# xingyizhou/CenterTrack

Hardware: AMD Instinct MI355X
Metric: frames/sec (DLA-34 + DCNv2 CenterTrack hot path: H2D of the frame + forward + decode + D2H + track association) (higher is better)
Workload: dtype f32; 1 GPU; mot17_512: mot heads, DLA-34, 512x512, 1 stream(s)/GPU, K=100, flip_test=False, seeded random-init weights; one step = 64 consecutive frames of every stream, each frame uploaded from pinned host memory inside the step (frame t+1 on a copy stream while frame t runs); global_batch=1, parallelism=streams sharded dp1, all-gather of packed detections, hip_graph=True

## Files before the change

centertrack_amd/_lib.py:

```python
import ctypes
import os

_PKG = os.path.dirname(os.path.abspath(__file__))
LIB_PATH = os.environ.get('CENTERTRACK_LIB') or os.path.join(_PKG, 'libcentertrack_hip.so')

c_float_p = ctypes.c_void_p
NUM_HEADS = 11
(HEAD_REG, HEAD_WH, HEAD_TRACKING, HEAD_LTRB, HEAD_LTRB_AMODAL, HEAD_DEP, HEAD_ROT, HEAD_DIM,
 HEAD_AMODEL_OFFSET, HEAD_NUSCENES_ATT, HEAD_VELOCITY) = range(NUM_HEADS)
HEAD_INDEX = {'reg': HEAD_REG, 'wh': HEAD_WH, 'tracking': HEAD_TRACKING, 'ltrb': HEAD_LTRB,
              'ltrb_amodal': HEAD_LTRB_AMODAL, 'dep': HEAD_DEP, 'rot': HEAD_ROT, 'dim': HEAD_DIM,
              'amodel_offset': HEAD_AMODEL_OFFSET, 'nuscenes_att': HEAD_NUSCENES_ATT,
              'velocity': HEAD_VELOCITY}
HEAD_CH = {'reg': 2, 'wh': 2, 'tracking': 2, 'ltrb': 4, 'ltrb_amodal': 4, 'dep': 1, 'rot': 8, 'dim': 3,
           'amodel_offset': 2, 'nuscenes_att': 8, 'velocity': 3}

CT_RELU = 1
CT_OUT_NCHW = 2
CT_DCN_MAIN, CT_DCN_FINISH, CT_DCN_OFFSETS = 1, 2, 4
CT_OK, CT_ERR_ARG, CT_ERR_LAUNCH, CT_ERR_WORKSPACE = 0, 1, 2, 3


class ConvDesc(ctypes.Structure):
    _fields_ = [('x', ctypes.c_void_p), ('N', ctypes.c_int), ('H', ctypes.c_int), ('W', ctypes.c_int),
                ('Cin', ctypes.c_int), ('ldx', ctypes.c_int),
                ('w_packed', ctypes.c_void_p), ('Cout', ctypes.c_int), ('ks', ctypes.c_int),
                ('stride', ctypes.c_int),
                ('scale', ctypes.c_void_p), ('shift', ctypes.c_void_p),
                ('res', ctypes.c_void_p), ('ldr', ctypes.c_int),
                ('y', ctypes.c_void_p), ('ldy', ctypes.c_int),
                ('flags', ctypes.c_int),
                ('sig_lo', ctypes.c_int), ('sig_hi', ctypes.c_int),
                ('dep_lo', ctypes.c_int), ('dep_hi', ctypes.c_int), ('depth_scale', ctypes.c_float),
                ('workspace', ctypes.c_void_p), ('workspace_bytes', ctypes.c_size_t),
                ('split_k', ctypes.c_int), ('algo', ctypes.c_int), ('w_winograd', ctypes.c_void_p),
                ('pool_y', ctypes.c_void_p), ('pool_ld', ctypes.c_int),
                ('proj_w_packed', ctypes.c_void_p), ('proj_scale', ctypes.c_void_p), ('proj_shift', ctypes.c_void_p),
                ('proj_y', ctypes.c_void_p), ('proj_ldy', ctypes.c_int)]


class DcnDesc(ctypes.Structure):
    _fields_ = [('x', ctypes.c_void_p), ('N', ctypes.c_int), ('H', ctypes.c_int), ('W', ctypes.c_int),
                ('Cin', ctypes.c_int), ('ldx', ctypes.c_int),
                ('om', ctypes.c_void_p), ('ldom', ctypes.c_int),
                ('w_packed', ctypes.c_void_p), ('Cout', ctypes.c_int),
                ('scale', ctypes.c_void_p), ('shift', ctypes.c_void_p),
                ('y', ctypes.c_void_p), ('ldy', ctypes.c_int),
                ('flags', ctypes.c_int),
                ('workspace', ctypes.c_void_p), ('workspace_bytes', ctypes.c_size_t),
                ('split_k', ctypes.c_int), ('algo', ctypes.c_int), ('fuse_offset', ctypes.c_int),
                ('w_off_packed', ctypes.c_void_p), ('b_off', ctypes.c_void_p),
                ('up_w', ctypes.c_void_p), ('up_f', ctypes.c_int), ('up_skip', ctypes.c_void_p), ('up_lds', ctypes.c_int),
                ('up_y', ctypes.c_void_p), ('up_ldy', ctypes.c_int),
                ('om_partial', ctypes.c_void_p), ('om_partial_bytes', ctypes.c_size_t),
                ('w_off_winograd', ctypes.c_void_p)]


CT_DCN_BWD_INPUT, CT_DCN_BWD_OFFSET_MASK, CT_DCN_BWD_WEIGHT = 1, 2, 4


class DcnBwdDesc(ctypes.Structure):
# ... 182 lines not shown
                ('inp_w', ctypes.c_int), ('inp_h', ctypes.c_int),
                ('host_rows', ctypes.c_void_p), ('rows_keep', ctypes.c_void_p),
                ('blob_params', ctypes.c_void_p), ('blob_counts', ctypes.c_void_p), ('blob_cap', ctypes.c_int),
                ('nslots', ctypes.c_int),
                ('graphs', ctypes.c_void_p * 3), ('frames', ctypes.c_void_p * 3),
                ('frame_bytes', ctypes.c_size_t),
                ('stream', ctypes.c_void_p),
                ('results', ctypes.c_void_p), ('results_cap', ctypes.c_int), ('done_flag', ctypes.c_void_p),
                ('pre', PrestageDesc)]


class FrameStepArgs(ctypes.Structure):
    _fields_ = [('slot', ctypes.c_int), ('frame_kind', ctypes.c_int),
                ('frame', ctypes.c_void_p), ('next_frame', ctypes.c_void_p),
                ('trans_input', ctypes.c_void_p), ('trans_inv', ctypes.c_void_p)]


CT_FRAME_DEVICE, CT_FRAME_HOST, CT_FRAME_IN_PLACE, CT_FRAME_UPLOADED = range(4)


ABI_VERSION = 103

EXPORTS = ['ct_last_error', 'ct_version', 'ct_set_tuning', 'ct_packed_weight_elems', 'ct_pack_conv_weight',
           'ct_packed_winograd_elems', 'ct_pack_winograd_weight', 'ct_conv2d',
           'ct_conv2d_workspace_bytes', 'ct_heads_fused', 'ct_dcn_v2', 'ct_dcn_v2_workspace_bytes', 'ct_dcn_v2_offsets_bytes', 'ct_dcn_v2_group', 'ct_dcn_v2_group_workspace_bytes', 'ct_dcn_v2_group_plan',
           'ct_dcn_v2_backward', 'ct_dcn_v2_backward_workspace_bytes', 'ct_packed_dcn_weight_t_elems', 'ct_pack_dcn_weight_t',
           'ct_generic_loss_forward', 'ct_generic_loss_backward', 'ct_generic_loss_workspace_bytes',
           'ct_conv2d_backward_weight', 'ct_conv2d_backward_weight_workspace_bytes', 'ct_heads_tail_backward',
           'ct_heads_tail_backward_workspace_bytes', 'ct_bn_stats', 'ct_bn_relu_apply', 'ct_bn_relu_backward', 'ct_bn_workspace_bytes',
           'ct_upsample_add_backward', 'ct_upsample_add_backward_workspace_bytes', 'ct_dcn_mask_sigmoid_backward',
           'ct_conv2d_s2_backward', 'ct_conv2d_s2_backward_workspace_bytes', 'ct_packed_conv_weight_s2t_elems', 'ct_pack_conv_weight_s2t',
           'ct_bn_act_apply', 'ct_bn_act_backward', 'ct_bn_act_workspace_bytes', 'ct_maxpool2x2_backward', 'ct_stem_forward',
           'ct_maxpool2x2', 'ct_upsample_add', 'ct_nchw_to_nhwc', 'ct_nhwc_to_nchw',
           'ct_decode_row_floats', 'ct_decode_workspace_bytes', 'ct_decode', 'ct_decode_pose_workspace_bytes',
           'ct_decode_pose', 'ct_render_pre_hm',
           'ct_tracker_create', 'ct_tracker_destroy', 'ct_tracker_reset', 'ct_tracker_num_tracks',
           'ct_tracker_id_count', 'ct_tracker_get_tracks', 'ct_tracker_step', 'ct_tracker_prehm_params', 'ct_linear_assignment', 'ct_tracker_set_mode', 'ct_tracker_init_tracks',
           'ct_tracker_step_public', 'ct_tracker_step_dets', 'ct_transform_points',
           'ct_preprocess_image', 'ct_preprocess_lut', 'ct_preprocess_device', 'ct_graph_begin', 'ct_graph_end', 'ct_graph_launch', 'ct_graph_destroy',
           'ct_memcpy_async', 'ct_memset_async', 'ct_stream_synchronize', 'ct_flip_merge', 'ct_flip_images',
           'ct_frame_loop_create', 'ct_frame_loop_destroy', 'ct_frame_loop_submit', 'ct_frame_loop_wait', 'ct_frame_loop_finish',
           'ct_frame_loop_finish_submit', 'ct_frame_loop_upload', 'ct_frame_loop_pending_slot', 'ct_frame_loop_in_flight',
           'ct_frame_loop_forget_upload', 'ct_frame_loop_prestage', 'ct_stem_forward_parts', 'ct_signal_host']

_lib = None


# ... 4 lines not shown
def load():
    global _lib
    if _lib is not None:
        return _lib
    if not os.path.exists(LIB_PATH):
        raise CTError('%s not found: build it with `python -c "import __graft_entry__ as g; g.build()"` '
                      '(hipcc --offload-arch=gfx950); there is no CPU fallback' % LIB_PATH)
    import torch
    lib = ctypes.CDLL(LIB_PATH)
    i, p, sz = ctypes.c_int, ctypes.c_void_p, ctypes.c_size_t
    lib.ct_last_error.restype = ctypes.c_char_p
    lib.ct_version.restype = i
    if lib.ct_version() != ABI_VERSION:
        raise CTError('%s is ABI version %d, this binding was written against %d: rebuild it (python -m '
                      'centertrack_amd.build)' % (LIB_PATH, lib.ct_version(), ABI_VERSION))
    lib.ct_set_tuning.argtypes = [ctypes.c_char_p, i]
    lib.ct_packed_weight_elems.restype = sz
    lib.ct_packed_weight_elems.argtypes = [i, i, i]
    lib.ct_pack_conv_weight.argtypes = [p, p, i, i, i, p]
    lib.ct_packed_winograd_elems.restype = sz
    lib.ct_packed_winograd_elems.argtypes = [i, i]
    lib.ct_pack_winograd_weight.argtypes = [p, p, i, i, p]
    lib.ct_conv2d.argtypes = [ctypes.POINTER(ConvDesc), p]
    lib.ct_conv2d_workspace_bytes.restype = sz
    lib.ct_conv2d_workspace_bytes.argtypes = [ctypes.POINTER(ConvDesc)]
    lib.ct_heads_fused.argtypes = [ctypes.POINTER(HeadsDesc), p]
    lib.ct_dcn_v2.argtypes = [ctypes.POINTER(DcnDesc), p]
    lib.ct_dcn_v2_workspace_bytes.restype = sz
    lib.ct_dcn_v2_workspace_bytes.argtypes = [ctypes.POINTER(DcnDesc)]
    lib.ct_dcn_v2_offsets_bytes.restype = sz
    lib.ct_dcn_v2_offsets_bytes.argtypes = [ctypes.POINTER(DcnDesc)]
    lib.ct_dcn_v2_group.argtypes = [ctypes.POINTER(DcnDesc), i, i, p]
    lib.ct_dcn_v2_group_workspace_bytes.restype = sz
    lib.ct_dcn_v2_group_workspace_bytes.argtypes = [ctypes.POINTER(DcnDesc)]
    lib.ct_dcn_v2_group_plan.argtypes = [ctypes.POINTER(DcnDesc), ctypes.POINTER(ctypes.c_size_t), ctypes.POINTER(ctypes.c_int)]
    lib.ct_dcn_v2_backward.argtypes = [ctypes.POINTER(DcnBwdDesc), p]
    lib.ct_dcn_v2_backward_workspace_bytes.restype = sz
    lib.ct_dcn_v2_backward_workspace_bytes.argtypes = [ctypes.POINTER(DcnBwdDesc)]
    lib.ct_packed_dcn_weight_t_elems.restype = sz
    lib.ct_packed_dcn_weight_t_elems.argtypes = [i, i]
    lib.ct_pack_dcn_weight_t.argtypes = [p, p, i, i, p]
    lib.ct_generic_loss_forward.argtypes = [ctypes.POINTER(LossDesc), p]
    lib.ct_generic_loss_backward.argtypes = [ctypes.POINTER(LossDesc), p]
    lib.ct_generic_loss_workspace_bytes.restype = sz
    lib.ct_generic_loss_workspace_bytes.argtypes = [ctypes.POINTER(LossDesc)]
    lib.ct_conv2d_backward_weight.argtypes = [ctypes.POINTER(ConvBwdWeightDesc), p]
# ... 124 lines not shown
```

centertrack_amd/csrc/conv_mfma.hip:

```cpp
#include "ct_common.h"
#define CT_KS_STAMP(i) CT_STAMP(i)
#include "ksplit_core.h"

CT_DEFINE_STAMPS(conv)

namespace {

struct ConvArgs {
    const float *x;
    const float *wp;
    int N, H, W, Cin, ldx;
    int tilesX, tilesY, coutBlocks, xcdPer;
    int NT;
    int nchunks;
    int chunksPerSplit;
    float *ws;
    int wsCout;
    EpiArgs epi;
    float *pool_y;
    int pool_ld;
    const float *proj_wp;
    EpiArgs epi2;
};

// ... 321 lines not shown
                const size_t Mtot = (size_t)a.N * a.epi.Ho * a.epi.Wo;
                float *wsp = a.ws + (size_t)split * Mtot * a.wsCout;
                const int co = (nt0 + nt) * 16 + li;
                if (oy < a.epi.Ho && co < a.wsCout) {
#pragma unroll
                    for (int e = 0; e < 4; ++e) {
                        const int ox = ox0 + lg * 4 + e;
                        if (ox < a.epi.Wo) wsp[(((size_t)n * a.epi.Ho + oy) * a.epi.Wo + ox) * a.wsCout + co] = sum[e];
                    }
                }
            } else {
                ct_store_tile(a.epi, sum, n, oy, ox0, (nt0 + nt) * 16, lane, psc[j], psh[j]);
            }
        };
    if constexpr (POOL && KS == 3 && STRIDE == 2) {
        auto fin_proj = [&](int mt, int nt, f32x4 sum, int j) {
            ct_store_tile(a.epi2, sum, n, oy0 + mt, ox0, (nt0 + nt) * 16, lane, psc2[j], psh2[j]);
        };
        ksplit_conv_tile<KS, STRIDE, WM, WN, WK, 2>(xin, a.H, a.W, a.ldx, a.Cin, a.wp, a.NT, nt0, oy0, ox0, c_begin, c_end, lds,
                                                    fin_main, hook, a.proj_wp, fin_proj);
    } else {
        ksplit_conv_tile<KS, STRIDE, WM, WN, WK, 2>(xin, a.H, a.W, a.ldx, a.Cin, a.wp, a.NT, nt0, oy0, ox0, c_begin, c_end, lds,
                                                    fin_main, hook);
    }
    CT_STAMP(6);
    CT_STAMP_RT(7);
}

__global__ __launch_bounds__(256) void splitk_reduce_kernel(const float *ws, int splits, size_t Mtot, int wsCout,
                                                            int N, EpiArgs e)
{
    const size_t idx = (size_t)blockIdx.x * 256 + threadIdx.x;
    const int quads = wsCout >> 2;
    if (idx >= Mtot * quads) return;
    const size_t m = idx / quads;
    const int c4 = (int)(idx - m * quads) << 2;
    f32x4 s = *reinterpret_cast<const f32x4 *>(ws + m * wsCout + c4);
    for (int k = 1; k < splits; ++k) {
        const f32x4 t = *reinterpret_cast<const f32x4 *>(ws + ((size_t)k * Mtot + m) * wsCout + c4);
        s += t;
    }
    const size_t hw = (size_t)e.Ho * e.Wo;
    const int n = (int)(m / hw);
    const size_t p = m - (size_t)n * hw;
#pragma unroll
    for (int i = 0; i < 4; ++i) {
// ... 246 lines not shown
extern "C" int ct_pack_conv_weight(const float *w_oihw, float *packed, int Cout, int Cin, int ks, void *stream)
{
    if (!w_oihw || !packed) CT_FAIL_ARG("ct_pack_conv_weight: null pointer");
    if (Cin % 16 || Cin <= 0 || Cout <= 0 || ks <= 0) CT_FAIL_ARG("ct_pack_conv_weight: Cin=%d must be a multiple of 16", Cin);
    const size_t total = ct_packed_weight_elems(Cout, Cin, ks);
    hipLaunchKernelGGL(pack_weight_kernel, dim3((unsigned)((total + 255) / 256)), dim3(256), 0, (hipStream_t)stream,
                       w_oihw, packed, Cout, Cin, ks, ct_cdiv(Cout, 16));
    CT_CHECK_LAUNCH("ct_pack_conv_weight");
    return CT_OK;
}

extern "C" size_t ct_conv2d_workspace_bytes(const ct_conv_desc *d)
{
    if (d && d->algo >= 201 && d->algo <= 211) return 0;
    Plan p;
    ct_conv_desc t = *d;
    float dummy;
    if (!t.workspace) t.workspace = &dummy;
    if (!t.y) t.y = &dummy;
    if (make_plan(&t, &p) != CT_OK) return 0;
    return ws_bytes(&t, p);
}

int ct_conv2d_winograd(const ct_conv_desc *d, void *stream);

extern "C" int ct_conv2d(const ct_conv_desc *d, void *stream)
{
    if (d && d->algo >= 201 && d->algo <= 211) {
        if (!d->x || !d->y) CT_FAIL_ARG("ct_conv2d: null pointer");
        if (d->ldx % 4 || ((uintptr_t)d->x & 15)) CT_FAIL_ARG("ct_conv2d: input view must be 16-byte aligned (ld %% 4 == 0)");
        return ct_conv2d_winograd(d, stream);
    }
    Plan p;
    int rc = make_plan(d, &p);
    if (rc != CT_OK) return rc;
    const size_t need = ws_bytes(d, p);
    if (need > 0 && (!d->workspace || d->workspace_bytes < need)) {
        ct_set_error("ct_conv2d: split_k=%d needs %zu workspace bytes, got %zu", p.splits, need, d->workspace_bytes);
        return CT_ERR_WORKSPACE;
    }
    if ((d->flags & CT_OUT_NCHW) && d->res) CT_FAIL_ARG("ct_conv2d: residual with NCHW output unsupported");
    ConvArgs a;
    a.x = d->x; a.wp = d->w_packed;
    a.N = d->N; a.H = d->H; a.W = d->W; a.Cin = d->Cin; a.ldx = d->ldx;
    a.tilesX = p.tilesX; a.tilesY = p.tilesY; a.coutBlocks = p.coutBlocks; a.xcdPer = ct_xcd_per(p.coutBlocks);
    a.NT = p.NT; a.nchunks = p.nchunks; a.chunksPerSplit = p.chunksPerSplit;
// ... 54 lines not shown
```

centertrack_amd/model.py:

```python
import ctypes
import os
from collections import OrderedDict

import torch

from . import _lib, autotune, ops
from .ops import View
from .weights import CHANNELS, LEVELS, dla34_param_shapes

BN_EPS = 1e-5
SMALL_SLOT_WGS = 600
FUSE_OFFSET = os.environ.get('CENTERTRACK_FUSE_OFFSET', '1') != '0'
WINOGRAD = os.environ.get('CENTERTRACK_WINOGRAD', '1') != '0'
FUSE_HEADS = os.environ.get('CENTERTRACK_FUSE_HEADS', '1') != '0'
FOLD_POOL = os.environ.get('CENTERTRACK_FOLD_POOL', '1') != '0'
FUSE_PROJ = os.environ.get('CENTERTRACK_FUSE_PROJ', '1') != '0'


def _fold_bn(sd, p):
    scale = sd[p + '.weight'].double() / torch.sqrt(sd[p + '.running_var'].double() + BN_EPS)
    shift = sd[p + '.bias'].double() - sd[p + '.running_mean'].double() * scale
    return scale.float().contiguous(), shift.float().contiguous()


class _Launch(object):
    __slots__ = ('fn', 'args', 'name', 'keep', 'us', 'ws_need')

    def __init__(self, name, fn, args, keep=(), reads=(), writes=(), us=5.0, ws_need=0):
        self.name, self.fn, self.args, self.keep = name, fn, args, keep
        self.us, self.ws_need = us, ws_need


class _DcnLayer(object):
    __slots__ = ('name', 'x', 'cout', 'out', 'up', 'main', 'finish', 'desc', 'fused', 'splits', 'use_ws', 'nkk')

    def __init__(self, name, x, cout, out, up):
        self.name, self.x, self.cout, self.out, self.up = name, x, cout, out, up


# ... 135 lines not shown
        w0 = torch.cat([sd[h + '.0.weight'] for h in self.heads], 0)
        P['head0_w'] = ops.pack_weight(w0)
        P['head0_ww'] = wino(w0)
        P['head0_b'] = torch.cat([sd[h + '.0.bias'] for h in self.heads], 0).contiguous()
        hc = self.head_conv
        ctot = sum(self.heads.values())
        w2 = torch.zeros((ctot, hc * len(self.heads), 1, 1), device=dev)
        c0 = 0
        for j, (h, c) in enumerate(self.heads.items()):
            w2[c0:c0 + c, hc * j:hc * (j + 1)] = sd[h + '.2.weight']
            c0 += c
        P['head2_w'] = ops.pack_weight(w2)
        P['head2_b'] = torch.cat([sd[h + '.2.bias'] for h in self.heads], 0).contiguous()
        for h in self.heads:
            P[h + '.2'] = (ops.pack_weight(sd[h + '.2.weight']), sd[h + '.2.bias'].contiguous())
        if hc == 256:
            for h, c in self.heads.items():
                if h in _lib.HEAD_INDEX:
                    P['sparse.' + h] = (ops.pack_weight(sd[h + '.0.weight']), sd[h + '.0.bias'].contiguous(),
                                        sd[h + '.2.weight'].reshape(c, hc).contiguous(), sd[h + '.2.bias'].contiguous())
        self._prepared = P
        return P

    def _build_plan(self, N, H, W, with_img, with_hm, fuse_sigmoid, sparse_heads=False, *, trunk_only=False):
        P = self._prepare()
        lib = _lib.load()
        dev = next(self.buffers()).device
        if H % 32 or W % 32:
            raise _lib.CTError('input %dx%d must be a multiple of 32 (reference pads to 32 too, opts.py:297)' % (H, W))
        plan = {'launches': [], 'ws_need': 0}
        L = plan['launches']
        tune = autotune.enabled()

        def alloc(h, w, c):
            return ops.new_view(N, h, w, c, dev)

        def add_conv(name, x, pk, cout, ks, stride=1, relu=True, res=None, out=None, **kw):
            wp, sc, sh, ww = pk
            d = ops.make_conv_desc(x, wp, cout, ks, stride, scale=sc, shift=sh, res=res, relu=relu, out=out,
                                   w_wino=(ww if stride == 1 else None), **kw)
            us = autotune.tune_conv(d, dev)[2] if tune else 10.0
            L.append(_Launch(name, 'conv', d, (x, res, out, pk, kw.get('out_nchw'), kw.get('pool'), kw.get('proj')), reads=(x, res),
                             writes=(out, kw.get('out_nchw')), us=us,
                             ws_need=lib.ct_conv2d_workspace_bytes(ctypes.byref(d))))
            return out

        x_in = torch.zeros((N, 3, H, W), device=dev)
        img_in = torch.zeros((N, 3, H, W), device=dev) if with_img else None
        hm_in = torch.zeros((N, 1, H, W), device=dev) if with_hm else None
        plan['inputs'] = (x_in, img_in, hm_in)
        s0 = alloc(H, W, 16)
        L.append(_Launch('stem', 'stem', (x_in, img_in, hm_in, s0), (), reads=(x_in, img_in, hm_in), writes=(s0,), us=46.0))
        l0 = add_conv('level0', s0, P['level0'], 16, 3, out=alloc(H, W, 16))
        l1 = add_conv('level1', l0, P['level1'], 32, 3, stride=2, out=alloc(H // 2, W // 2, 32))

        def leaf(name, x, pk, cin, cout, stride, R, out, bottom=None, level_root=False, make_bottom=False):
            h, w = x.H // stride, x.W // stride
            fold = None
            fuse_proj = FUSE_PROJ and stride == 2 and cin != cout
            if stride > 1 and bottom is None:
                if level_root:
                    bottom = R.slice(2 * cout, cin)
                    make_bottom = True
                elif not fuse_proj:
                    bottom = alloc(h, w, cin)
                    make_bottom = True
            elif stride == 1:
                bottom = x
            if stride > 1 and make_bottom:
                if FOLD_POOL:
                    fold = bottom
                else:
                    L.append(_Launch(name + '.pool', 'pool', (x, bottom), reads=(x,), writes=(bottom,)))
            t = alloc(h, w, cout)
            x1 = R.slice(cout, cout)
            x2 = R.slice(0, cout)
            if fuse_proj:
# ... 38 lines not shown
        def deform(name, x, cout, out, up=None):
            dcn_layers.append(_DcnLayer(name, x, cout, out, up))
            return out

        def ida(p, layers, startp, endp, o, up_f):
            for i in range(startp + 1, endp):
                k = i - startp
                f = up_f[k]
                xi = layers[i]
                up = alloc(xi.H * f, xi.W * f, o)
                deform('%s.proj_%d' % (p, k), xi, o, alloc(xi.H, xi.W, o),
                       up=(P['%s.up_%d' % (p, k)], f, layers[i - 1], up))
                layers[i] = deform('%s.node_%d' % (p, k), up, o, alloc(up.H, up.W, o))

        layers = list(feats)
        outs = [layers[-1]]
        ida('dla_up.ida_0', layers, 4, 6, 256, [1, 2]); outs.insert(0, layers[-1])
        ida('dla_up.ida_1', layers, 3, 6, 128, [1, 2, 2]); outs.insert(0, layers[-1])
        ida('dla_up.ida_2', layers, 2, 6, 64, [1, 2, 2, 2]); outs.insert(0, layers[-1])
        y = [outs[0], outs[1], outs[2]]
        ida('ida_up', y, 0, 3, 64, [1, 2, 4])
        feat = y[-1]
        plan['feat'] = feat
        produced0 = {id(f_.buf): 0 for f_ in feats}
        knobs, dcn_launches = self._tune_dcn_schedule(dcn_layers, produced0, N, H, W, dev, tune)
        plan['dcn_knobs'] = knobs
        plan['dcn_layers'] = {ly.name: (ly.up[3] if ly.up is not None else ly.out) for ly in dcn_layers}
        L.extend(dcn_launches)

        small, big = P['heads_small'], P['heads_big']
        plan['sparse'] = None
        if sparse_heads:
            sp = [h for h in self.heads if ('sparse.' + h) in P]
            if {'ltrb', 'ltrb_amodal'} & set(self.heads):
                sp = [h for h in sp if h not in ('reg', 'wh')]
            if not sp or 'hm' not in self.heads or {'hps', 'hm_hp'} & set(self.heads) or not fuse_sigmoid:
                raise _lib.CTError('sparse heads need an hm head, regression heads with head_conv 256, no pose heads '
                                   'and the detector\'s fused epilogues')
            plan['sparse'] = {'feat': feat, 'heads': [(h,) + P['sparse.' + h] for h in sp], 'depth_scale': self.depth_scale}
            small = [h for h in small if ('sparse.' + h) not in P]
            if any(('sparse.' + h) in P for h in big):
                raise _lib.CTError('sparse heads: %s do not fit the fused-heads launch' % [h for h in big if ('sparse.' + h) in P])
        if trunk_only:
            if sparse_heads:
                raise _lib.CTError('a trunk-only plan has no heads, sparse or dense')
            outputs = OrderedDict()
        elif small or plan['sparse'] is not None:
# ... 89 lines not shown
                us = autotune.tune_conv(d, dev)[2] if tune else 7.0
                L.append(_Launch('heads.%s.2' % h, 'conv', d, (mid, o), us=us,
                                 ws_need=lib.ct_conv2d_workspace_bytes(ctypes.byref(d))))
                outputs[h] = o
        return OrderedDict((h, outputs[h]) for h in self.heads if h in outputs)

    def run_stem_partial(self, x, pre_img, out):
        P = self._prepare()
        lib = _lib.load()
        w = P['stem_w']
        rc = lib.ct_stem_forward_parts(x.data_ptr(), ops._p(pre_img), None, None, 0, x.shape[0], x.shape[2], x.shape[3],
                                       w[0].data_ptr(), ops._p(w[1]) if pre_img is not None else None, None,
                                       P['stem_scale'].data_ptr(), P['stem_shift'].data_ptr(), out.ptr, out.ld,
                                       _lib.stream_ptr())
        if rc != 0:
            _lib.check(rc, 'stem (x / pre_img terms)')

    def _run_plan(self, plan, inputs=None, stem_partial=None, launches=None):
        P = self._prepared
        lib = _lib.load()
        st = _lib.stream_ptr()
        for l in (plan['launches'] if launches is None else launches):
            if l.fn == 'conv':
                rc = lib.ct_conv2d(ctypes.byref(l.args), st)
            elif l.fn == 'dcn_group':
                arr, n, phases = l.args
                rc = lib.ct_dcn_v2_group(arr, n, phases, st)
            elif l.fn == 'heads':
                rc = lib.ct_heads_fused(ctypes.byref(l.args), st)
            elif l.fn == 'pool':
                x, y = l.args
                rc = lib.ct_maxpool2x2(x.ptr, x.N, x.H, x.W, x.C, x.ld, y.ptr, y.ld, st)
            elif l.fn == 'stem':
                x, img, hm, y = l.args
                if inputs is not None:
                    x, img, hm = inputs
                w = P['stem_w']
                if stem_partial is not None:
                    if hm is None:
                        raise _lib.CTError('a split stem needs the pre_hm input')
                    rc = lib.ct_stem_forward_parts(None, None, hm.data_ptr(), stem_partial.ptr, stem_partial.ld,
                                                   x.shape[0], x.shape[2], x.shape[3], None, None, w[2].data_ptr(),
                                                   P['stem_scale'].data_ptr(), P['stem_shift'].data_ptr(), y.ptr, y.ld, st)
                    if rc != 0:
                        _lib.check(rc, l.name)
                    continue
                rc = lib.ct_stem_forward(x.data_ptr(), ops._p(img), ops._p(hm), x.shape[0], x.shape[2], x.shape[3],
# ... 222 lines not shown
                    print('dcn schedule N=%d %dx%d knobs %s: %d launches, %.1f us (%.1f without)' % (N, H, W, knobs, len(launches), us, us0))
                if us < best[0]:
                    best = (us, knobs)
            del launches
        autotune._CACHE[key] = tuple(best[1]) + (round(best[0], 1),)
        autotune._save_file()
        return best[1], self._schedule_dcn(layers, produced0, N, dev, best[1])

    @staticmethod
    def plan_signature(plan):
        parts = ['dcn_knobs=%s' % (tuple(plan.get('dcn_knobs', ())),)]
        for l in plan['launches']:
            if l.fn == 'conv':
                parts.append('%s:conv:%d:%d' % (l.name, int(l.args.algo), int(l.args.split_k)))
            elif l.fn == 'dcn_group':
                arr, n, phases = l.args
                parts.append('%s:dcn:%d:%s' % (l.name, phases, ','.join(
                    '%d/%d/%d' % (int(arr[j].algo), int(arr[j].split_k), int(arr[j].fuse_offset)) for j in range(n))))
            else:
                parts.append('%s:%s' % (l.name, l.fn))
        return ';'.join(parts)

    def get_plan(self, N, H, W, with_img, with_hm, fuse_sigmoid=False, sparse_heads=False, *, trunk_only=False):
        key = (N, H, W, with_img, with_hm, fuse_sigmoid, sparse_heads, trunk_only)
        if key not in self._plans:
            self._plans[key] = self._build_plan(*key[:7], trunk_only=trunk_only)
        return self._plans[key]

    def forward_plan(self, plan, x, pre_img=None, pre_hm=None):
        xi, ii, hi = plan['inputs']
        xi.copy_(x)
        if ii is not None:
            ii.copy_(pre_img)
        if hi is not None:
            hi.copy_(pre_hm)
        self._run_plan(plan)
        return plan['outputs']

    @torch.no_grad()
    def forward(self, x, pre_img=None, pre_hm=None, fuse_sigmoid=False):
        if pre_img is not None and not self.pre_img:
            raise _lib.CTError('model was built with pre_img=False')
        if pre_hm is not None and not self.pre_hm:
            raise _lib.CTError('model was built with pre_hm=False')
        N, _, H, W = x.shape
        plan = self.get_plan(N, H, W, pre_img is not None, pre_hm is not None, fuse_sigmoid)
        out = self.forward_plan(plan, x, pre_img, pre_hm)
        z = OrderedDict((k, v.clone()) for k, v in out.items())
        if self.model_output_list:
# ... 54 lines not shown
```

centertrack_amd/ops.py:

```python
import ctypes

import torch

from . import _lib
from ._lib import CT_OUT_NCHW, CT_RELU, ConvDesc, DcnBwdDesc, DcnDesc, DecodeDesc


class View(object):
    __slots__ = ('buf', 'c0', 'C')

    def __init__(self, buf, c0=0, C=None):
        assert buf.dim() == 4 and buf.is_contiguous() and buf.dtype == torch.float32
        self.buf = buf
        self.c0 = c0
        self.C = buf.shape[3] - c0 if C is None else C
        assert 0 <= c0 and c0 + self.C <= buf.shape[3]

    N = property(lambda s: s.buf.shape[0])
    H = property(lambda s: s.buf.shape[1])
    W = property(lambda s: s.buf.shape[2])
    ld = property(lambda s: s.buf.shape[3])
    ptr = property(lambda s: s.buf.data_ptr() + 4 * s.c0)

    def slice(self, c0, C):
# ... 65 lines not shown
        d.y, d.ldy = out_nchw.data_ptr(), 0
        flags |= CT_OUT_NCHW
    else:
        d.y, d.ldy = out.ptr, out.ld
    d.flags = flags
    d.sig_lo, d.sig_hi = sig
    d.dep_lo, d.dep_hi = dep
    d.depth_scale = depth_scale
    if workspace is not None:
        d.workspace, d.workspace_bytes = workspace.data_ptr(), workspace.numel() * workspace.element_size()
    d.split_k = split_k
    d.algo = algo
    if w_wino is not None:
        d.w_winograd = w_wino.data_ptr()
    if pool is not None:
        assert ks == 3 and stride == 2 and (pool.N, pool.H, pool.W, pool.C) == (x.N, x.H // 2, x.W // 2, x.C)
        d.pool_y, d.pool_ld = pool.ptr, pool.ld
    if proj is not None:
        pw, psc, psh, py = proj
        assert ks == 3 and stride == 2 and (py.N, py.H, py.W, py.C) == (x.N, x.H // 2, x.W // 2, Cout)
        d.proj_w_packed, d.proj_scale, d.proj_shift = pw.data_ptr(), _p(psc), _p(psh)
        d.proj_y, d.proj_ldy = py.ptr, py.ld
    return d


def conv2d(x, wp, Cout, ks, stride=1, out=None, **kw):
    lib = _lib.load()
    pad = ks // 2
    Ho = (x.H + 2 * pad - ks) // stride + 1
    Wo = (x.W + 2 * pad - ks) // stride + 1
    if out is None and kw.get('out_nchw') is None:
        out = new_view(x.N, Ho, Wo, Cout, x.buf.device, ld=(Cout + 3) // 4 * 4)
    d = make_conv_desc(x, wp, Cout, ks, stride, out=out, **kw)
    if d.workspace is None and kw.get('split_k', 0) != 1:
        need = lib.ct_conv2d_workspace_bytes(ctypes.byref(d))
        if need:
            ws = torch.empty(need // 4, dtype=torch.float32, device=x.buf.device)
            d.workspace, d.workspace_bytes = ws.data_ptr(), need
            kw['_keep'] = ws
    _lib.check(lib.ct_conv2d(ctypes.byref(d), _lib.stream_ptr()), 'ct_conv2d')
    return out if out is not None else kw['out_nchw']


def make_dcn_desc(x, om, wp, Cout, scale, shift, relu, out, workspace=None, split_k=0, algo=0, w_off=None,
                  b_off=None, up=None, om_partial=None, raw_offsets=False, w_off_wino=None):
    d = DcnDesc()
# ... 672 lines not shown
```

include/centertrack_hip.h:

```cpp
#ifndef CENTERTRACK_HIP_H
#define CENTERTRACK_HIP_H

#include <stddef.h>
#include <stdint.h>

#ifdef __cplusplus
extern "C" {
#endif

#define CT_OK 0
#define CT_ERR_ARG 1
#define CT_ERR_LAUNCH 2
#define CT_ERR_WORKSPACE 3

#define CT_RELU 1
#define CT_OUT_NCHW 2

#define CT_ABI_VERSION 103

const char *ct_last_error(void);
int ct_version(void);
int ct_set_tuning(const char *key, int value);

size_t ct_packed_weight_elems(int Cout, int Cin, int ks);
int ct_pack_conv_weight(const float *w_oihw, float *packed, int Cout, int Cin, int ks, void *stream);
size_t ct_packed_winograd_elems(int Cout, int Cin);
int ct_pack_winograd_weight(const float *w_oihw, float *packed, int Cout, int Cin, void *stream);

typedef struct ct_conv_desc {
    const float *x; int N, H, W, Cin, ldx;
    const float *w_packed; int Cout, ks, stride;
    const float *scale; const float *shift;
    const float *res; int ldr;
    float *y; int ldy;
    int flags;
    int sig_lo, sig_hi;
    int dep_lo, dep_hi; float depth_scale;
    float *workspace; size_t workspace_bytes;
    int split_k;
    int algo;
    const float *w_winograd;
    float *pool_y; int pool_ld;
    const float *proj_w_packed; const float *proj_scale; const float *proj_shift;
    float *proj_y; int proj_ldy;
} ct_conv_desc;
int ct_conv2d(const ct_conv_desc *d, void *stream);
size_t ct_conv2d_workspace_bytes(const ct_conv_desc *d);

#define CT_MAX_FUSED_HEADS 8
typedef struct ct_heads_desc {
    const float *x; int N, H, W, Cin, ldx;
    const float *w0_winograd; const float *b0;
    int nheads;
    const float *w2; const float *b2;
    int cout[CT_MAX_FUSED_HEADS], coff[CT_MAX_FUSED_HEADS];
    float *out; int ctot;
    int sig_lo, sig_hi, dep_lo, dep_hi; float depth_scale;
} ct_heads_desc;
int ct_heads_fused(const ct_heads_desc *d, void *stream);

typedef struct ct_dcn_desc {
    const float *x; int N, H, W, Cin, ldx;
    const float *om; int ldom;
    const float *w_packed; int Cout;
    const float *scale; const float *shift;
    float *y; int ldy;
    int flags;
    float *workspace; size_t workspace_bytes;
    int split_k;
    int algo;
// ... 321 lines not shown
```

Before: 1152 frames/s.

## Fuse level0 and level1 convolutions into one tiled kernel with LDS intermediate

Adds a fused kernel that computes the stride-1 16->16 level0 conv on a halo tile in LDS, then immediately runs the stride-2 level1 conv from that LDS tile, writing only level1 output. This removes the full-resolution level0 activation round trip through global memory and one launch. In exchange it recomputes halo pixels, uses large LDS per block (limiting occupancy), and only applies when level0 has no other reader.

```diff
diff --git a/centertrack_amd/_lib.py b/centertrack_amd/_lib.py
--- a/centertrack_amd/_lib.py
+++ b/centertrack_amd/_lib.py
@@ -37,6 +37,11 @@
                 ('pool_y', ctypes.c_void_p), ('pool_ld', ctypes.c_int),
                 ('proj_w_packed', ctypes.c_void_p), ('proj_scale', ctypes.c_void_p), ('proj_shift', ctypes.c_void_p),
                 ('proj_y', ctypes.c_void_p), ('proj_ldy', ctypes.c_int)]
+
+
+class FrontDesc(ConvDesc):
+    _fields_ = [('pre_w_packed', ctypes.c_void_p), ('pre_scale', ctypes.c_void_p), ('pre_shift', ctypes.c_void_p),
+                ('pre_flags', ctypes.c_int)]
 
 
 class DcnDesc(ctypes.Structure):
@@ -265,7 +270,7 @@
 ABI_VERSION = 103
 
 EXPORTS = ['ct_last_error', 'ct_version', 'ct_set_tuning', 'ct_packed_weight_elems', 'ct_pack_conv_weight',
-           'ct_packed_winograd_elems', 'ct_pack_winograd_weight', 'ct_conv2d',
+           'ct_packed_winograd_elems', 'ct_pack_winograd_weight', 'ct_conv2d', 'ct_conv2d_front',
            'ct_conv2d_workspace_bytes', 'ct_heads_fused', 'ct_dcn_v2', 'ct_dcn_v2_workspace_bytes', 'ct_dcn_v2_offsets_bytes', 'ct_dcn_v2_group', 'ct_dcn_v2_group_workspace_bytes', 'ct_dcn_v2_group_plan',
            'ct_dcn_v2_backward', 'ct_dcn_v2_backward_workspace_bytes', 'ct_packed_dcn_weight_t_elems', 'ct_pack_dcn_weight_t',
            'ct_generic_loss_forward', 'ct_generic_loss_backward', 'ct_generic_loss_workspace_bytes',
@@ -316,6 +321,7 @@
     lib.ct_packed_winograd_elems.argtypes = [i, i]
     lib.ct_pack_winograd_weight.argtypes = [p, p, i, i, p]
     lib.ct_conv2d.argtypes = [ctypes.POINTER(ConvDesc), p]
+    lib.ct_conv2d_front.argtypes = [ctypes.POINTER(FrontDesc), p]
     lib.ct_conv2d_workspace_bytes.restype = sz
     lib.ct_conv2d_workspace_bytes.argtypes = [ctypes.POINTER(ConvDesc)]
     lib.ct_heads_fused.argtypes = [ctypes.POINTER(HeadsDesc), p]
diff --git a/centertrack_amd/csrc/conv_mfma.hip b/centertrack_amd/csrc/conv_mfma.hip
--- a/centertrack_amd/csrc/conv_mfma.hip
+++ b/centertrack_amd/csrc/conv_mfma.hip
@@ -367,6 +367,189 @@
     } else {
         ksplit_conv_tile<KS, STRIDE, WM, WN, WK, 2>(xin, a.H, a.W, a.ldx, a.Cin, a.wp, a.NT, nt0, oy0, ox0, c_begin, c_end, lds,
                                                     fin_main, hook);
+    }
+    CT_STAMP(6);
+    CT_STAMP_RT(7);
+}
+
+struct FrontArgs {
+    const float *x, *wp0, *wp1;
+    int N, H, W, ldx;
+    int tilesX, tilesY;
+    int NT1;
+    EpiArgs epi0;
+    EpiArgs epi1;
+};
+
+template <int TH>
+struct FrontCfg {
+    static constexpr int IH = 2 * TH + 1, IW = 33, IP = IH * IW;
+    static constexpr int MT0 = (IP + 15) / 16;
+    static constexpr int PH = IH + 2, PW = IW + 2, PP = PH * PW;
+    static constexpr int PATCH = PP * 16, INTER = MT0 * 256;
+    static constexpr size_t LDS_BYTES = (size_t)(PATCH + INTER) * sizeof(float);
+};
+
+template <int TH>
+__global__ __launch_bounds__(256) void front_fused_kernel(FrontArgs a)
+{
+    using C = FrontCfg<TH>;
+    static_assert(TH % 4 == 0, "level1 rows are dealt to 4 waves");
+    extern __shared__ __attribute__((aligned(16))) float lds[];
+    float *patch = lds, *inter = lds + C::PATCH;
+    CT_STAMP_RT(0);
+    CT_STAMP(1);
+    CT_STAMP_HW(8);
+    const int tid = threadIdx.x;
+    const int lane = tid & 63;
+    const int wave = __builtin_amdgcn_readfirstlane(tid >> 6);
+    const int li = lane & 15, lg = lane >> 4;
+    int bid = blockIdx.x;
+    const int tx = bid % a.tilesX; bid /= a.tilesX;
+    const int ty = bid % a.tilesY; bid /= a.tilesY;
+    const int n = bid;
+    const int oy0 = ty * TH, ox0 = tx * 16;
+    const int y0 = 2 * oy0 - 1, x0 = 2 * ox0 - 1;
+    const int iy0 = y0 - 1, ix0 = x0 - 1;
+
+    constexpr int RP = (C::PP + 63) / 64;
+    const int sq = tid & 3, sslot = tid >> 2;
+    const __amdgpu_buffer_rsrc_t xrs = __builtin_amdgcn_make_buffer_rsrc(
+        const_cast<float *>(a.x + (size_t)n * a.H * a.W * a.ldx), 0, (int)((((unsigned)a.H * a.W - 1u) * a.ldx + 16) * 4u), 0x00020000);
+    f32x4 stage[RP];
+#pragma unroll
+    for (int j = 0; j < RP; ++j) {
+        const int P = sslot + 64 * j;
+        const int py = P / C::PW, px = P - py * C::PW;
+        const int iy = iy0 + py, ix = ix0 + px;
+        const int goff = (P < C::PP && iy >= 0 && iy < a.H && ix >= 0 && ix < a.W) ? ((iy * a.W + ix) * a.ldx + sq * 4) * 4 : (int)0x80000000;
+        stage[j] = __builtin_bit_cast(f32x4, __builtin_amdgcn_raw_buffer_load_b128(xrs, goff, 0, 0));
+    }
+    const __amdgpu_buffer_rsrc_t wrs0 = __builtin_amdgcn_make_buffer_rsrc(const_cast<float *>(a.wp0), 0, 9 << 10, 0x00020000);
+    f32x4 b0[9];
+#pragma unroll
+    for (int tap = 0; tap < 9; ++tap)
+        b0[tap] = __builtin_bit_cast(f32x4, __builtin_amdgcn_raw_buffer_load_b128(wrs0, lane << 4, tap << 10, 0));
+    float sc0, sh0;
+    ct_load_scale_shift(a.epi0, 0, lane, sc0, sh0);
+    const __amdgpu_buffer_rsrc_t wrs1 = __builtin_amdgcn_make_buffer_rsrc(const_cast<float *>(a.wp1), 0, (9 * a.NT1) << 10, 0x00020000);
+    f32x4 b1[9][2];
+    float psc[2], psh[2];
+    auto load_b1 = [&](int nb) {
+#pragma unroll
+        for (int nt = 0; nt < 2; ++nt) {
+            const int vo = (min(nb * 2 + nt, a.NT1 - 1) << 10) + (lane << 4);
+#pragma unroll
+            for (int tap = 0; tap < 9; ++tap)
+                b1[tap][nt] = __builtin_bit_cast(f32x4, __builtin_amdgcn_raw_buffer_load_b128(wrs1, vo, (tap * a.NT1) << 10, 0));
+            ct_load_scale_shift(a.epi1, (nb * 2 + nt) * 16, lane, psc[nt], psh[nt]);
+        }
+    };
+    CT_STAMP(2);
+#pragma unroll
+    for (int j = 0; j < RP; ++j) {
+        const int P = sslot + 64 * j;
+        if (P < C::PP) *reinterpret_cast<f32x4 *>(patch + P * 16 + ((sq ^ ((P >> 1) & 2)) << 2)) = stage[j];
+    }
+    load_b1(0);
+    __syncthreads();
+    CT_STAMP(3);
+
+    constexpr int TPW = (C::MT0 + 3) / 4;
+    constexpr int G = 3;
+#pragma unroll 1
+    for (int g0 = 0; g0 < TPW; g0 += G) {
+        f32x4 acc[G];
+        int pb[G];
+#pragma unroll
+        for (int j = 0; j < G; ++j) {
+            const int p = min((wave + 4 * (g0 + j)) * 16 + li, C::IP - 1);
+            const int row = p / C::IW;
+            pb[j] = row * C::PW + (p - row * C::IW);
+            acc[j] = f32x4{0.f, 0.f, 0.f, 0.f};
+        }
+#pragma unroll
+        for (int tap = 0; tap < 9; ++tap) {
+            f32x4 af[G];
+#pragma unroll
+            for (int j = 0; j < G; ++j) {
+                const int P = pb[j] + (tap / 3) * C::PW + (tap % 3);
+                af[j] = *reinterpret_cast<const f32x4 *>(patch + P * 16 + ((lg ^ ((P >> 1) & 2)) << 2));
+            }
+#pragma unroll
+            for (int e = 0; e < 4; ++e)
+#pragma unroll
+                for (int j = 0; j < G; ++j)
+                    acc[j] = __builtin_amdgcn_mfma_f32_16x16x4f32(af[j][e], b0[tap][e], acc[j], 0, 0, 0);
+        }
+#pragma unroll
+        for (int j = 0; j < G; ++j) {
+            const int t = wave + 4 * (g0 + j);
+            if (t >= C::MT0) continue;
+#pragma unroll
+            for (int e = 0; e < 4; ++e) {
+                const int p = t * 16 + lg * 4 + e;
+                const int row = p / C::IW, col = p - row * C::IW;
+                const int yy = y0 + row, xx = x0 + col;
+                float v = ct_epilogue_plain(a.epi0, acc[j][e], sc0, sh0, 0.0f);
+                if (yy < 0 || yy >= a.H || xx < 0 || xx >= a.W) v = 0.0f;
+                inter[p * 16 + (((li >> 2) ^ ((p >> 1) & 2)) << 2) + (li & 3)] = v;
+            }
+        }
+    }
+    __syncthreads();
+    CT_STAMP(4);
+
+    constexpr int WM = TH / 4;
+    int pbase[WM];
+#pragma unroll
+    for (int mt = 0; mt < WM; ++mt) pbase[mt] = ((wave * WM + mt) * 2) * C::IW + li * 2;
+#pragma unroll 1
+    for (int nb = 0; nb * 2 < a.NT1; ++nb) {
+        f32x4 acc[WM][2];
+#pragma unroll
+        for (int mt = 0; mt < WM; ++mt)
+#pragma unroll
+            for (int nt = 0; nt < 2; ++nt) acc[mt][nt] = f32x4{0.f, 0.f, 0.f, 0.f};
+#pragma unroll
+        for (int tap = 0; tap < 9; ++tap) {
+            f32x4 af[WM];
+#pragma unroll
+            for (int mt = 0; mt < WM; ++mt) {
+                const int P = pbase[mt] + (tap / 3) * C::IW + (tap % 3);
+                af[mt] = *reinterpret_cast<const f32x4 *>(inter + P * 16 + ((lg ^ ((P >> 1) & 2)) << 2));
+            }
+#pragma unroll
+            for (int e = 0; e < 4; ++e)
+#pragma unroll
+                for (int mt = 0; mt < WM; ++mt)
+#pragma unroll
+                    for (int nt = 0; nt < 2; ++nt)
+                        acc[mt][nt] = __builtin_amdgcn_mfma_f32_16x16x4f32(af[mt][e], b1[tap][nt][e], acc[mt][nt], 0, 0, 0);
+        }
+        if (nb == 0) CT_STAMP(5);
+        const float sc[2] = {psc[0], psc[1]}, sh[2] = {psh[0], psh[1]};
+        if ((nb + 1) * 2 < a.NT1) load_b1(nb + 1);
+        const unsigned img = (unsigned)a.epi1.Ho * a.epi1.Wo;
+        const __amdgpu_buffer_rsrc_t yrs = __builtin_amdgcn_make_buffer_rsrc(
+            a.epi1.y + (size_t)n * img * a.epi1.ldy, 0, (int)(((img - 1u) * a.epi1.ldy + a.epi1.Cout) * 4u), 0x00020000);
+        const int xr = ox0 + (lg << 2);
+#pragma unroll
+        for (int mt = 0; mt < WM; ++mt) {
+            const int oy = oy0 + wave * WM + mt;
+            if (oy >= a.epi1.Ho) continue;
+#pragma unroll
+            for (int nt = 0; nt < 2; ++nt) {
+                const int co = (nb * 2 + nt) * 16 + li;
+                const int vy = ((oy * a.epi1.Wo + xr) * a.epi1.ldy + co) * 4;
+#pragma unroll
+                for (int i = 0; i < 4; ++i) {
+                    const float v = ct_epilogue_plain(a.epi1, acc[mt][nt][i], sc[nt], sh[nt], 0.0f);
+                    __builtin_amdgcn_raw_buffer_store_b32(__float_as_uint(v), yrs, (co < a.epi1.Cout && xr + i < a.epi1.Wo) ? vy : (int)0x80000000,
+                                                          i * a.epi1.ldy * 4, 0);
+                }
+            }
+        }
     }
     CT_STAMP(6);
     CT_STAMP_RT(7);
@@ -659,6 +842,59 @@
     return ws_bytes(&t, p);
 }
 
+namespace {
+template <int TH>
+int launch_front(const FrontArgs &a, int Ho, hipStream_t s)
+{
+    using C = FrontCfg<TH>;
+    static_assert(C::LDS_BYTES <= 160 * 1024, "LDS regions too large");
+    FrontArgs b = a;
+    b.tilesY = ct_cdiv(Ho, TH);
+    const long blocks = (long)b.N * b.tilesX * b.tilesY;
+    if (blocks > 0x7fffffffL) CT_FAIL_ARG("ct_conv2d_front: grid too large");
+    auto k = front_fused_kernel<TH>;
+    static bool attr_set = false;
+    if (!attr_set && C::LDS_BYTES > 48 * 1024) {
+        (void)hipFuncSetAttribute(reinterpret_cast<const void *>(k), hipFuncAttributeMaxDynamicSharedMemorySize, (int)C::LDS_BYTES);
+        attr_set = true;
+    }
+    hipLaunchKernelGGL(k, dim3((unsigned)blocks), dim3(256), C::LDS_BYTES, s, b);
+    return CT_OK;
+}
+}
+
+extern "C" int ct_conv2d_front(const ct_front_desc *f, void *stream)
+{
+    if (!f || !f->conv.x || !f->conv.w_packed || !f->conv.y || !f->pre_w_packed) CT_FAIL_ARG("ct_conv2d_front: null pointer");
+    const ct_conv_desc *d = &f->conv;
+    if (d->ks != 3 || d->stride != 2 || d->Cin != 16 || d->Cout <= 0 || d->Cout % 16)
+        CT_FAIL_ARG("ct_conv2d_front: conv3x3 16 -> 16 followed by conv3x3 stride 2 16 -> 16 k (got ks=%d stride=%d Cin=%d Cout=%d)",
+                    d->ks, d->stride, d->Cin, d->Cout);
+    if (d->N <= 0 || d->H <= 0 || d->W <= 0) CT_FAIL_ARG("ct_conv2d_front: bad shape");
+    if (d->ldx % 4 || d->ldx < 16 || ((uintptr_t)d->x & 15)) CT_FAIL_ARG("ct_conv2d_front: input view must be 16-byte aligned (ld %% 4 == 0)");
+    if (d->ldy < d->Cout) CT_FAIL_ARG("ct_conv2d_front: output pitch %d < Cout", d->ldy);
+    if (d->res || (d->flags & ~CT_RELU) || (f->pre_flags & ~CT_RELU) || d->sig_hi > d->sig_lo || d->dep_hi > d->dep_lo || d->pool_y ||
+        d->proj_w_packed || d->split_k > 1)
+        CT_FAIL_ARG("ct_conv2d_front: scale / shift / ReLU epilogues on NHWC only (no residual, side output, transform or split-K)");
+    if (d->algo != 0) CT_FAIL_ARG("ct_conv2d_front: algo %d (there is one launch shape: 0)", d->algo);
+    FrontArgs a;
+    a.x = d->x; a.wp0 = f->pre_w_packed; a.wp1 = d->w_packed;
+    a.N = d->N; a.H = d->H; a.W = d->W; a.ldx = d->ldx;
+    const int Ho = (d->H - 1) / 2 + 1, Wo = (d->W - 1) / 2 + 1;
+    a.tilesX = ct_cdiv(Wo, 16); a.tilesY = 0;
+    a.NT1 = d->Cout / 16;
+    a.epi1.scale = d->scale; a.epi1.shift = d->shift; a.epi1.res = nullptr; a.epi1.y = d->y;
+    a.epi1.ldr = 0; a.epi1.ldy = d->ldy; a.epi1.Cout = d->Cout; a.epi1.Ho = Ho; a.epi1.Wo = Wo;
+    a.epi1.flags = d->flags; a.epi1.sig_lo = a.epi1.sig_hi = a.epi1.dep_lo = a.epi1.dep_hi = 0; a.epi1.depth_scale = 0.0f;
+    a.epi0 = a.epi1;
+    a.epi0.scale = f->pre_scale; a.epi0.shift = f->pre_shift; a.epi0.y = nullptr; a.epi0.ldy = 0; a.epi0.Cout = 16;
+    a.epi0.Ho = d->H; a.epi0.Wo = d->W; a.epi0.flags = f->pre_flags;
+    const int rc = launch_front<8>(a, Ho, (hipStream_t)stream);
+    if (rc != CT_OK) return rc;
+    CT_CHECK_LAUNCH("ct_conv2d_front");
+    return CT_OK;
+}
+
 int ct_conv2d_winograd(const ct_conv_desc *d, void *stream);
 
 extern "C" int ct_conv2d(const ct_conv_desc *d, void *stream)
diff --git a/centertrack_amd/model.py b/centertrack_amd/model.py
--- a/centertrack_amd/model.py
+++ b/centertrack_amd/model.py
@@ -15,6 +15,20 @@
 FUSE_HEADS = os.environ.get('CENTERTRACK_FUSE_HEADS', '1') != '0'
 FOLD_POOL = os.environ.get('CENTERTRACK_FOLD_POOL', '1') != '0'
 FUSE_PROJ = os.environ.get('CENTERTRACK_FUSE_PROJ', '1') != '0'
+
+
+def fuse_front_enabled():
+    return os.environ.get('CENTERTRACK_FUSE_FRONT', '1') != '0'
+
+
+def front_fusable(d0, d1, level0_readers):
+    def plain(d):
+        return (int(d.flags) == _lib.CT_RELU and not d.res and not d.pool_y and not d.proj_w_packed
+                and d.sig_hi <= d.sig_lo and d.dep_hi <= d.dep_lo)
+    return (level0_readers == 1 and plain(d0) and plain(d1)
+            and (d0.ks, d0.stride, d0.Cin, d0.Cout) == (3, 1, 16, 16)
+            and (d1.ks, d1.stride, d1.Cin) == (3, 2, 16) and d1.Cout > 0 and d1.Cout % 16 == 0
+            and d1.x == d0.y and d1.ldx == d0.ldy and (d1.N, d1.H, d1.W) == (d0.N, d0.H, d0.W))
 
 
 def _fold_bn(sd, p):
@@ -196,7 +210,9 @@
         self._prepared = P
         return P
 
-    def _build_plan(self, N, H, W, with_img, with_hm, fuse_sigmoid, sparse_heads=False, *, trunk_only=False):
+    def _build_plan(self, N, H, W, with_img, with_hm, fuse_sigmoid, sparse_heads=False, *, trunk_only=False, fuse_front=None):
+        if fuse_front is None:
+            fuse_front = fuse_front_enabled()
         P = self._prepare()
         lib = _lib.load()
         dev = next(self.buffers()).device
@@ -225,8 +241,23 @@
         plan['inputs'] = (x_in, img_in, hm_in)
         s0 = alloc(H, W, 16)
         L.append(_Launch('stem', 'stem', (x_in, img_in, hm_in, s0), (), reads=(x_in, img_in, hm_in), writes=(s0,), us=46.0))
-        l0 = add_conv('level0', s0, P['level0'], 16, 3, out=alloc(H, W, 16))
-        l1 = add_conv('level1', l0, P['level1'], 32, 3, stride=2, out=alloc(H // 2, W // 2, 32))
+        level0_readers = 1 + (0 if (fuse_sigmoid or trunk_only) else 1)
+        l1 = alloc(H // 2, W // 2, 32)
+        fused_front = False
+        if fuse_front:
+            l0p = ops.View(s0.buf.new_empty((1, 1, 1, 16)), 0, 16)
+            d0 = ops.make_conv_desc(s0, P['level0'][0], 16, 3, 1, scale=P['level0'][1], shift=P['level0'][2], relu=True, out=l0p)
+            d1 = ops.make_conv_desc(l0p, P['level1'][0], 32, 3, 2, scale=P['level1'][1], shift=P['level1'][2], relu=True, out=l1)
+            d1.N, d1.H, d1.W = N, H, W
+            fused_front = front_fusable(d0, d1, level0_readers)
+        if fused_front:
+            pk0, pk1 = P['level0'], P['level1']
+            d = ops.make_front_desc(s0, (pk0[0], pk0[1], pk0[2], True), pk1[0], 32, scale=pk1[1], shift=pk1[2], relu=True, out=l1)
+            L.append(_Launch('level0+level1', 'conv', d, (s0, None, l1, pk0, pk1), reads=(s0,), writes=(l1,), us=18.0))
+            l0 = None
+        else:
+            l0 = add_conv('level0', s0, P['level0'], 16, 3, out=alloc(H, W, 16))
+            add_conv('level1', l0, P['level1'], 32, 3, stride=2, out=l1)
 
         def leaf(name, x, pk, cin, cout, stride, R, out, bottom=None, level_root=False, make_bottom=False):
             h, w = x.H // stride, x.W // stride
@@ -311,7 +342,7 @@
         ida('ida_up', y, 0, 3, 64, [1, 2, 4])
         feat = y[-1]
         plan['feat'] = feat
-        produced0 = {id(f_.buf): 0 for f_ in feats}
+        produced0 = {id(f_.buf): 0 for f_ in feats if f_ is not None}
         knobs, dcn_launches = self._tune_dcn_schedule(dcn_layers, produced0, N, H, W, dev, tune)
         plan['dcn_knobs'] = knobs
         plan['dcn_layers'] = {ly.name: (ly.up[3] if ly.up is not None else ly.out) for ly in dcn_layers}
@@ -447,7 +478,10 @@
         st = _lib.stream_ptr()
         for l in (plan['launches'] if launches is None else launches):
             if l.fn == 'conv':
-                rc = lib.ct_conv2d(ctypes.byref(l.args), st)
+                if isinstance(l.args, _lib.FrontDesc):
+                    rc = lib.ct_conv2d_front(ctypes.byref(l.args), st)
+                else:
+                    rc = lib.ct_conv2d(ctypes.byref(l.args), st)
             elif l.fn == 'dcn_group':
                 arr, n, phases = l.args
                 rc = lib.ct_dcn_v2_group(arr, n, phases, st)
@@ -716,9 +750,9 @@
         return ';'.join(parts)
 
     def get_plan(self, N, H, W, with_img, with_hm, fuse_sigmoid=False, sparse_heads=False, *, trunk_only=False):
-        key = (N, H, W, with_img, with_hm, fuse_sigmoid, sparse_heads, trunk_only)
+        key = (N, H, W, with_img, with_hm, fuse_sigmoid, sparse_heads, trunk_only, fuse_front_enabled())
         if key not in self._plans:
-            self._plans[key] = self._build_plan(*key[:7], trunk_only=trunk_only)
+            self._plans[key] = self._build_plan(*key[:7], trunk_only=trunk_only, fuse_front=key[8])
         return self._plans[key]
 
     def forward_plan(self, plan, x, pre_img=None, pre_hm=None):
diff --git a/centertrack_amd/ops.py b/centertrack_amd/ops.py
--- a/centertrack_amd/ops.py
+++ b/centertrack_amd/ops.py
@@ -111,6 +111,29 @@
         d.proj_w_packed, d.proj_scale, d.proj_shift = pw.data_ptr(), _p(psc), _p(psh)
         d.proj_y, d.proj_ldy = py.ptr, py.ld
     return d
+
+
+def make_front_desc(x, pre, wp, Cout, scale=None, shift=None, relu=True, out=None):
+    pw, psc, psh, prelu = pre
+    assert x.C == 16 and (out.N, out.H, out.W, out.C) == (x.N, (x.H - 1) // 2 + 1, (x.W - 1) // 2 + 1, Cout)
+    d = _lib.FrontDesc()
+    d.x, d.N, d.H, d.W, d.Cin, d.ldx = x.ptr, x.N, x.H, x.W, x.C, x.ld
+    d.w_packed, d.Cout, d.ks, d.stride = wp.data_ptr(), Cout, 3, 2
+    d.scale, d.shift = _p(scale), _p(shift)
+    d.y, d.ldy = out.ptr, out.ld
+    d.flags = CT_RELU if relu else 0
+    d.split_k, d.algo = 1, 0
+    d.pre_w_packed, d.pre_scale, d.pre_shift = pw.data_ptr(), _p(psc), _p(psh)
+    d.pre_flags = CT_RELU if prelu else 0
+    return d
+
+
+def conv2d_front(x, pre, wp, Cout, out=None, **kw):
+    if out is None:
+        out = new_view(x.N, (x.H - 1) // 2 + 1, (x.W - 1) // 2 + 1, Cout, x.buf.device)
+    d = make_front_desc(x, pre, wp, Cout, out=out, **kw)
+    _lib.check(_lib.load().ct_conv2d_front(ctypes.byref(d), _lib.stream_ptr()), 'ct_conv2d_front')
+    return out
 
 
 def conv2d(x, wp, Cout, ks, stride=1, out=None, **kw):
diff --git a/include/centertrack_hip.h b/include/centertrack_hip.h
--- a/include/centertrack_hip.h
+++ b/include/centertrack_hip.h
@@ -46,6 +46,13 @@
 } ct_conv_desc;
 int ct_conv2d(const ct_conv_desc *d, void *stream);
 size_t ct_conv2d_workspace_bytes(const ct_conv_desc *d);
+
+typedef struct ct_front_desc {
+    ct_conv_desc conv;
+    const float *pre_w_packed; const float *pre_scale; const float *pre_shift;
+    int pre_flags;
+} ct_front_desc;
+int ct_conv2d_front(const ct_front_desc *d, void *stream);
 
 #define CT_MAX_FUSED_HEADS 8
 typedef struct ct_heads_desc {
```

Measured after the change: 1185 frames/s (median of 4 runs). 1.03x the previous value.
